# kobigurk/phase2-bn254

Measured on AMD Instinct MI355X. Metric: BN254 G1 MSM throughput (Mscalar-mul/s) at 2^26 points, higher is better.
Workload: dtype u32x8 (256-bit Montgomery limbs)

## Files before the change

phase2-bn254_amd/csrc/msm_common.hpp:

```cpp
#pragma once
#include <stdint.h>

namespace zk {

constexpr uint32_t SIGN_BIT = 0x80000000u;

struct MsmGeom {
  uint32_t c;
  uint32_t W;
  uint32_t nb;
  uint8_t width[64];
  uint8_t shift[64];
  uint32_t rmul;
  uint32_t rshift;
};

constexpr uint32_t MSM_SIZE_BINS = 4096;
constexpr uint32_t PART_THREADS = 1024;
constexpr uint32_t PART_MAX_ST = 16384;
constexpr uint32_t PART_MAX_EB = PART_MAX_ST / PART_THREADS;
constexpr uint32_t PART_LO_MAX = 12;
constexpr uint32_t PART_EC = 32;
constexpr uint32_t PART_LDS_A = 76 * 1024;
constexpr uint32_t PART_LDS_MAX = 160 * 1024 - 512;
constexpr uint32_t KEY_NONE_MASK = 0x00ffffffu;

struct PartGeom {
  uint32_t lo_bits;
  uint32_t nbin;
  uint32_t st;
  uint32_t n_st;
  uint32_t n_chunk;
  uint32_t rows_per_chunk;
};

constexpr uint32_t BIG_SEG = PART_EC * PART_THREADS;

struct BigPlan {
  uint32_t n_big;
  uint32_t total_seg;
};

constexpr uint32_t MSM_HEAVY_BLOCKS = 65536;
constexpr uint32_t MSM_HEAVY_SEG = 4096;
constexpr uint32_t MSM_HEAVY_LANES = 64;
constexpr uint32_t MSM_PAIR_MAX_BUCKETS = 3u << 17;

constexpr uint32_t MSM_FINAL_MAX = 1024;
constexpr uint32_t MSM_TREE_SLICE = 512;
constexpr uint32_t MSM_MAX_LEVELS = 8;
constexpr uint32_t MSM_MAX_JOBS = MSM_MAX_LEVELS + 24;

}
```

phase2-bn254_amd/csrc/msm_host.hpp:

```cpp
#pragma once
#include <atomic>
#include <chrono>
#include <cstring>
#include <map>
#include <mutex>
#include <type_traits>
#include <vector>

#include "msm_impl.hpp"
#include "msm_join.hpp"
#include "msm_partition.hpp"
#include "msm_plan.hpp"
#include "msm_pools.hpp"

namespace zk {

namespace {

std::mutex g_part_cfg_mu;
std::map<int, int> g_part_cfg;
template <class F>
int part_configure(int dev) {
  std::lock_guard<std::mutex> lk(g_part_cfg_mu);
  auto it = g_part_cfg.find(dev);
  if (it != g_part_cfg.end()) return it->second;
  int rc = zk::part_configure(dev);
  hipError_t e = hipFuncSetAttribute(reinterpret_cast<const void*>(msm_tree_kernel<F>), hipFuncAttributeMaxDynamicSharedMemorySize, 160 * 1024);
  if (e != hipSuccess) {
    std::fprintf(stderr, "[mi355zk] hipFuncSetAttribute(partition kernel, 160 KiB LDS) failed: %s\n", hipGetErrorString(e));
    rc = ZK_ERR_DEVICE;
  }
  g_part_cfg[dev] = rc;
  return rc;
}

template <class F>
struct MsmWs : MsmPartWs {
  XYZZ<F>*seg_sums, *buckets, *partA, *partS, *rc, *wsums, *sumtmp;
  static_assert(sizeof(XYZZ<F>) == (sizeof(F) == sizeof(Fq) ? 128 : 256), "msm_plan.hpp sizes the record regions by these");
  MsmWs(char* ws, const MsmLayout& L) : MsmPartWs(ws, L) {
    at(ws, seg_sums, L.seg_sums), at(ws, buckets, L.buckets), at(ws, partA, L.partA), at(ws, partS, L.partS), at(ws, rc, L.rc), at(ws, wsums, L.wsums);
    at(ws, sumtmp, L.sumtmp);
  }
};

template <class F>
struct MsmCall : MsmPartCall {
  MsmWs<F> ws;
  bool dense;
};

template <class Fn>
void with_a4_carry(bool a4, bool carry, Fn&& fn) {
  auto with_carry = [&](auto A4) { if (carry) fn(A4, std::true_type{}); else fn(A4, std::false_type{}); };
  if (a4) with_carry(std::true_type{}); else with_carry(std::false_type{});
}

struct HeavyParams {
  uint32_t hb, heavy, seg, grid;
  int dense, carry;
};
template <class F>
int launch_heavy(hipStream_t st, const Affine<F>* bases, const uint32_t* vals, const uint32_t* first, const uint32_t* last, const uint32_t* order,
                 const uint32_t* sizes_b, uint32_t* item_off, XYZZ<F>* seg_sums, XYZZ<F>* buckets, unsigned long long* d_err, const HeavyParams& H) {
  launch_heavy_plan(st, sizes_b, H.hb, H.heavy, H.seg, item_off);
  ZK_HIP(hipGetLastError());
  hipLaunchKernelGGL(msm_accumulate_heavy_kernel<F>, dim3(H.grid), dim3(MSM_HEAVY_LANES), MSM_HEAVY_LANES * sizeof(typename BucketAcc<F>::type), st, bases, vals,
                     first, last, order, item_off, H.hb, H.seg, seg_sums, H.dense, d_err);
  ZK_HIP(hipGetLastError());
  hipLaunchKernelGGL(msm_heavy_combine_kernel<F>, dim3(H.hb < 2048 ? H.hb : 2048), dim3(64), 64 * sizeof(typename BucketAcc<F>::type), st, seg_sums, order, item_off,
                     H.hb, buckets, H.carry);
  ZK_HIP(hipGetLastError());
  return ZK_OK;
}

template <class F>
int launch_accumulate(const MsmCall<F>& A, const ChunkPlan& C, const Affine<F>* bases_set, bool carry) {
  constexpr bool g2 = std::is_same<F, Fq2>::value;
  const MsmWs<F>& W = A.ws;
  const MsmKnobs& K = A.knobs;
  const hipStream_t st = A.st;
  const uint32_t n_buckets = A.plan.n_buckets;
// ... 18 lines not shown
  const bool pair = pair_mode < 0 ? n_buckets <= MSM_PAIR_MAX_BUCKETS : pair_mode != 0;
  const bool w2 = g2 && !pair && (K.g2_waves == 0 ? g_msm_inflight[A.dev & 15].load(std::memory_order_relaxed) <= 1 : K.g2_waves == 2);
  with_a4_carry(K.acc_a4, carry, [&](auto A4, auto CARRY) {
    constexpr bool a4 = decltype(A4)::value, cy = decltype(CARRY)::value;
    auto go = [&](auto kern, dim3 g) {
      hipLaunchKernelGGL(kern, g, block, 0, st, bases_set, W.vals_b, W.first, W.last, W.order, skip_len, skip_hb, n_buckets, W.buckets, dense, W.d_err);
    };
    if constexpr (g2) {
      if (pair) go(msm_accumulate_pair_kernel<a4, cy>, pgrid);
      else if (w2) go(msm_accumulate_g2w2_kernel<a4, cy>, grid);
      else go(msm_accumulate_kernel<F, a4, cy>, grid);
    } else {
      if (pair) go(msm_accumulate_pair_g1_kernel<a4, cy>, pgrid);
      else go(msm_accumulate_kernel<F, a4, cy>, grid);
    }
  });
  ZK_HIP(hipGetLastError());
  prof_end(msm_slots().acc, st);
  if (msm_checkpoint(A, "accumulate", C)) return (int)ZK_ERR_DEVICE;
  return ZK_OK;
}

template <class F>
int launch_reduce(const MsmCall<F>& A) {
  const MsmPlan& P = A.plan;
  const MsmWs<F>& W = A.ws;
  const hipStream_t st = A.st;
  const uint32_t WL = P.WL, n_levels = P.n_levels, n_out = P.n_out, t_rows = P.t_rows, t_cols = P.t_cols;
  TreeJobs<F> J{};
  J.quad = A.knobs.quad_tail ? 1u : 0u;
  const XYZZ<F>* in = W.buckets;
  uint64_t o = 0;
  for (uint32_t lv = 0; lv < n_levels; ++lv) {
    uint32_t threads = P.lvl_chunks[lv] * WL;
    XYZZ<F>* LA = W.partA + o * WL;
    XYZZ<F>* LS = W.partS + o * WL;
    if (A.knobs.quad_tail && threads <= A.knobs.quad_max_chunks)
      hipLaunchKernelGGL(msm_reduce_level_quad_kernel<F>, dim3((4 * threads + 255) / 256), dim3(256), 0, st, in, P.lvl_cnt[lv], 1u << P.lvl_logl[lv],
                         lv == 0 ? 1u : 0u, WL, LA, LS);
    else
      hipLaunchKernelGGL(msm_reduce_level_kernel<F>, dim3((threads + 255) / 256), dim3(256), 0, st, in, P.lvl_cnt[lv], 1u << P.lvl_logl[lv],
                         lv == 0 ? 1u : 0u, WL, LA, LS);
    ZK_HIP(hipGetLastError());
    J.in[lv] = LA;
    J.cnt[lv] = J.stride[lv] = P.lvl_chunks[lv];
    J.bit[lv] = -1;
    in = LS;
    o += P.lvl_chunks[lv];
  }
  auto plain = [&J](uint32_t j) { J.reps[j] = 1; J.rep_stride[j] = 0; J.elem_stride[j] = 1; J.limit[j] = 0xffffffffu; J.off[j] = 0; };
  for (uint32_t lv = 0; lv < n_levels; ++lv) plain(lv);
  uint32_t n_jobs = n_levels;
  if (!P.tail2d) {
    for (uint32_t j = 0; j < P.final_bits; ++j, ++n_jobs) {
      plain(n_jobs);
      J.in[n_jobs] = in;
      J.cnt[n_jobs] = J.stride[n_jobs] = P.final_cnt;
      J.bit[n_jobs] = (int32_t)j;
      J.off[n_jobs] = P.final_off;
    }
  } else {
    J.in[n_jobs] = in; J.cnt[n_jobs] = t_cols; J.stride[n_jobs] = P.final_cnt; J.bit[n_jobs] = -1; J.off[n_jobs] = 0;
    J.reps[n_jobs] = t_rows; J.rep_stride[n_jobs] = t_cols; J.elem_stride[n_jobs] = 1; J.limit[n_jobs] = P.final_cnt;
    ++n_jobs;
    J.in[n_jobs] = in; J.cnt[n_jobs] = t_rows; J.stride[n_jobs] = P.final_cnt; J.bit[n_jobs] = -1; J.off[n_jobs] = 0;
    J.reps[n_jobs] = t_cols; J.rep_stride[n_jobs] = 1; J.elem_stride[n_jobs] = t_cols; J.limit[n_jobs] = P.final_cnt;
    ++n_jobs;
  }
  const size_t lds = 256 * sizeof(typename BucketAcc<F>::type);
  XYZZ<F>* dst = W.sumtmp;
  for (uint32_t launch = 0;; ++launch) {
    const bool families = P.tail2d && launch == 0;
    uint32_t left = 1;
    uint64_t o_dst = 0;
    for (uint32_t j = 0; j < n_jobs; ++j) {
      const uint32_t sl = (J.cnt[j] + MSM_TREE_SLICE - 1) / MSM_TREE_SLICE;
      J.first_block[j + 1] = J.first_block[j] + J.reps[j] * sl;
      if (sl > left) left = sl;
    }
    const bool last = left == 1 && !families;
    for (uint32_t j = 0; j < n_jobs; ++j) {
      const uint32_t sl = (J.cnt[j] + MSM_TREE_SLICE - 1) / MSM_TREE_SLICE;
      if (families && j >= n_levels) {
        J.out[j] = W.rc + (j == n_levels ? 0 : t_rows);
        J.out_w[j] = t_rows + t_cols;
      } else if (last) {
        J.out[j] = W.wsums + j;
        J.out_w[j] = n_out;
      } else {
        J.out[j] = dst + o_dst;
        J.out_w[j] = 1;
        o_dst += (uint64_t)WL * sl;
      }
    }
    J.n_jobs = n_jobs;
    hipLaunchKernelGGL(msm_tree_kernel<F>, dim3(J.first_block[n_jobs] * WL), dim3(256), lds, st, J);
    ZK_HIP(hipGetLastError());
    if (last) break;
    for (uint32_t j = 0; j < (families ? n_levels : n_jobs); ++j) {
      const uint32_t sl = (J.cnt[j] + MSM_TREE_SLICE - 1) / MSM_TREE_SLICE;
      J.in[j] = J.out[j];
      J.cnt[j] = J.stride[j] = sl;
      J.bit[j] = -1;
      plain(j);
    }
    if (families) {
      n_jobs = n_levels;
      for (uint32_t j = 0; j < P.final_bits; ++j, ++n_jobs) {
        plain(n_jobs);
        J.in[n_jobs] = W.rc + t_rows;
        J.cnt[n_jobs] = t_cols;
        J.stride[n_jobs] = t_rows + t_cols;
        J.bit[n_jobs] = (int32_t)j;
        J.off[n_jobs] = P.final_off;
      }
      for (uint32_t j = 0; j < P.row_bits; ++j, ++n_jobs) {
        plain(n_jobs);
        J.in[n_jobs] = W.rc;
        J.cnt[n_jobs] = t_rows;
        J.stride[n_jobs] = t_rows + t_cols;
        J.bit[n_jobs] = (int32_t)j;
      }
    }
    dst = dst == W.sumtmp ? W.sumtmp + (uint64_t)WL * P.tree_tmp : W.sumtmp;
  }
  return ZK_OK;
}

template <class F>
int msm_finish_set(const MsmCall<F>& A, SmallWsLease& lease, std::unique_lock<std::mutex>& lk, const Affine<F>* d_bases, const uint32_t* d_sc_first,
                   Jacobian<F>* result, bool last_set, long long* err_index_out) {
  const MsmPlan& P = A.plan;
  const hipStream_t st = A.st;
// ... 62 lines not shown
  if (top) ZK_HIP(hipMemcpyAsync(T.vals.data(), A.ws.vals_b, (size_t)top * 4, hipMemcpyDeviceToHost, A.st));
  ZK_HIP(hipStreamSynchronize(A.st));
  return ZK_OK;
}

template <class F>
int msm_device(const Affine<F>* d_bases, uint64_t n_bases, uint64_t base_offset, const uint32_t* d_scalars, uint64_t n,
               const uint32_t* d_density, const uint32_t* d_dprefix, hipStream_t st, Jacobian<F>* out, long long* err_index_out,
               bool dense = false, const Affine<F>* d_bases2 = nullptr, Jacobian<F>* out2 = nullptr, uint32_t wgroups = 1,
               uint32_t wgroup = 0, bool scalars_mont = false, MsmChunks* chunks = nullptr, uint64_t table_stride = 0, uint32_t table_c = 0) {
  *out = Jacobian<F>::zero();
  if (out2) *out2 = Jacobian<F>::zero();
  *err_index_out = -1;
  if (n == 0) return ZK_OK;
  if (n_bases > 0x7fffffffull || n > 0x7fffffffull) return ZK_ERR_BAD_ARGS;
  int dev = 0;
  ZK_HIP(hipGetDevice(&dev));
  struct Inflight {
    std::atomic<int>& c;
    explicit Inflight(std::atomic<int>& x) : c(x) { c.fetch_add(1, std::memory_order_relaxed); }
    ~Inflight() { c.fetch_sub(1, std::memory_order_relaxed); }
  } inflight(g_msm_inflight[dev & 15]);
  const MsmKnobs K = msm_knobs();
  MsmRequest R;
  R.group = (int)(sizeof(F) / sizeof(Fq));
  R.n = n;
  R.base_offset = base_offset;
  R.wgroups = wgroups;
  R.wgroup = wgroup;
  if (chunks) R.n_chunks = chunks->n_chunks, R.cuts = chunks->cuts;
  R.two_sets = d_bases2 != nullptr;
  R.table_stride = table_stride;
  R.table_c = table_c;
  const MsmPlan P = msm_plan(R, K);
  if (P.rc) return P.rc;

  int rc = part_configure<F>(dev);
  if (rc) return rc;
  Workspace& dev_ws = ws_of(dev);
  std::unique_lock<std::mutex> lk(dev_ws.mu, std::defer_lock);
  void* base = nullptr;
  SmallWsLease lease;
  if (P.L.total_bytes <= WS_SMALL) {
    rc = tws_acquire(dev, P.L.total_bytes, st, &lease, &base);
  } else {
    lk.lock();
    rc = ws_reserve(dev_ws, P.L.total_bytes, &base);
  }
  if (rc) return rc;
  const MsmCall<F> A{{P, K, R.group, dev, st, n, base_offset, table_stride, d_density, d_dprefix, scalars_mont}, MsmWs<F>((char*)base, P.L), dense};
  ZK_HIP(hipMemsetAsync(A.ws.d_err, 0xff, 16, st));
  lease.idle = false;

  const uint32_t* d_sc_first = d_scalars;
  for (uint32_t c = 0; c < (uint32_t)P.chunks.size(); ++c) {
    const ChunkPlan& C = P.chunks[c];
    const uint32_t* d_sc = d_scalars;
    if (chunks) {
      const void* p = nullptr;
      rc = chunks->acquire(c, st, &p);
      if (rc) return rc;
      d_sc = (const uint32_t*)p;
    }
    d_sc_first = d_sc;
    rc = launch_digits(A, A.ws, C, d_sc);
    if (rc == ZK_OK && chunks) rc = chunks->digits_enqueued(c, st);
    if (rc == ZK_OK) rc = launch_partition(A, A.ws, C);
    if (rc == ZK_OK) rc = launch_accumulate(A, C, d_bases, c > 0);
    if (rc) return rc;
  }
  if (g_msm_bucket_tap) {
    if (P.chunks.size() != 1) return ZK_ERR_BAD_ARGS;
    if (int trc = msm_tap_buckets(A, *g_msm_bucket_tap)) return trc;
  }
  const bool two_sets = d_bases2 != nullptr && out2 != nullptr;
  rc = msm_finish_set(A, lease, lk, d_bases, d_sc_first, out, !two_sets, err_index_out);
  if (rc != ZK_OK || !two_sets) return rc;
  lease.idle = false;
  rc = launch_accumulate(A, P.chunks[0], d_bases2, false);
  if (rc) return rc;
  return msm_finish_set(A, lease, lk, d_bases, d_sc_first, out2, true, err_index_out);
}

// ... 52 lines not shown
```

phase2-bn254_amd/csrc/msm_impl.hpp:

```cpp
#pragma once
#include <hip/hip_runtime.h>

#include <type_traits>

#include "curveu.hpp"
#include "device_util.hpp"
#include "msm_common.hpp"

namespace zk {

namespace {

template <class F>
__device__ __forceinline__ Affine<F> load_affine(const Affine<F>* p) {
  Affine<F> r;
  const uint4* q = reinterpret_cast<const uint4*>(p);
  uint4* d = reinterpret_cast<uint4*>(&r);
#pragma unroll
  for (int i = 0; i < (int)(sizeof(Affine<F>) / 16); ++i) d[i] = q[i];
  return r;
}

template <class T>
__device__ __forceinline__ void store_vec(T* p, const T& v) {
// ... 287 lines not shown
    const Affine<Fq2>* __restrict__ bases, const uint32_t* __restrict__ vals, const uint32_t* __restrict__ first, const uint32_t* __restrict__ last,
    const uint32_t* __restrict__ order, uint32_t heavy, uint32_t hb, uint32_t n_buckets, XYZZ<Fq2>* __restrict__ buckets, int skip_zero,
    unsigned long long* __restrict__ err_base) {
  accumulate_pair_body<Fq2, A4, CARRY>(bases, vals, first, last, order, heavy, hb, n_buckets, buckets, skip_zero, err_base);
}
template <bool A4, bool CARRY>
__global__ void __launch_bounds__(256) msm_accumulate_pair_g1_kernel(
    const Affine<Fq>* __restrict__ bases, const uint32_t* __restrict__ vals, const uint32_t* __restrict__ first, const uint32_t* __restrict__ last,
    const uint32_t* __restrict__ order, uint32_t heavy, uint32_t hb, uint32_t n_buckets, XYZZ<Fq>* __restrict__ buckets, int skip_zero,
    unsigned long long* __restrict__ err_base) {
  accumulate_pair_body<Fq, A4, CARRY>(bases, vals, first, last, order, heavy, hb, n_buckets, buckets, skip_zero, err_base);
}

template <class F>
__global__ void __launch_bounds__(256) __attribute__((amdgpu_waves_per_eu(1, 2))) msm_accumulate_split_kernel(
    const Affine<F>* __restrict__ bases, const uint32_t* __restrict__ vals, const uint32_t* __restrict__ first, const uint32_t* __restrict__ last,
    const uint32_t* __restrict__ order, uint32_t split_t, uint32_t heavy, uint32_t heavy_hb, uint32_t hb, XYZZ<F>* __restrict__ buckets,
    int skip_zero, unsigned long long* __restrict__ err_base) {
  using U = typename BucketAcc<F>::type;
  const uint32_t gt = blockIdx.x * blockDim.x + threadIdx.x, i = gt >> 2, role = gt & 3u;
  if (i >= hb) return;
  const uint32_t b = order[i];
  const uint32_t j = first[b], e = last[b];
  if (e - j <= split_t || (e - j > heavy && i < heavy_hb)) return;
  U part = xyzzr_load(XYZZ<F>::zero());
  if (j + role < e) part = xyzzr_load(xyzzu_to_r(accumulate_run<F, false>(U::zero(), bases, vals, j + role, e, 4, skip_zero != 0, err_base)));
  const U p0 = quad_fetch<0>(part), p1 = quad_fetch<1>(part), p2 = quad_fetch<2>(part), p3 = quad_fetch<3>(part);
  const U sum = xyzzr_add_quad(xyzzr_add_quad(p0, p1, role), xyzzr_add_quad(p2, p3, role), role);
  if (role == 0) store_vec(buckets + b, xyzzr_store(sum));
}

template <class F>
__global__ void __launch_bounds__(256) msm_reduce_level_kernel(const XYZZ<F>* __restrict__ in, uint32_t count, uint32_t L, uint32_t off,
                                                              uint32_t W, XYZZ<F>* __restrict__ outA, XYZZ<F>* __restrict__ outS) {
  uint32_t chunks = (count + L - 1) / L;
  uint32_t t = blockIdx.x * blockDim.x + threadIdx.x;
  if (t >= chunks * W) return;
  uint32_t w = t / chunks, ch = t % chunks;
  uint32_t lo = ch * L, hi = lo + L < count ? lo + L : count;
  const XYZZ<F>* B = in + (uint64_t)w * count;
  uint32_t steps = 2 * (hi - lo);
  auto run = xyzzr_load(XYZZ<F>::zero()), acc = run;
  for (uint32_t it = 0; it < steps; ++it) {
    uint32_t x = hi - 1 - (it >> 1);
    bool do_acc = ((it & 1) != 0) == (off != 0);
    auto a = do_acc ? acc : run;
    auto b = do_acc ? run : xyzzr_load(load_vec(B + x));
    xyzzr_add(a, b);
    if (do_acc) acc = a;
    else run = a;
  }
  store_vec(outA + t, xyzzr_store(acc));
  store_vec(outS + t, xyzzr_store(run));
}

template <class F>
__global__ void __launch_bounds__(256) __attribute__((amdgpu_waves_per_eu(1, 2))) msm_reduce_level_quad_kernel(const XYZZ<F>* __restrict__ in, uint32_t count, uint32_t L, uint32_t off,
                                                                   uint32_t W, XYZZ<F>* __restrict__ outA, XYZZ<F>* __restrict__ outS) {
  const uint32_t chunks = (count + L - 1) / L;
  const uint32_t gt = blockIdx.x * blockDim.x + threadIdx.x, t = gt >> 2, role = gt & 3u;
  if (t >= chunks * W) return;
  const uint32_t w = t / chunks, ch = t % chunks;
  const uint32_t lo = ch * L, hi = lo + L < count ? lo + L : count;
  const XYZZ<F>* B = in + (uint64_t)w * count;
  auto run = xyzzr_load(XYZZ<F>::zero()), acc = run;
  for (uint32_t x = hi; x-- > lo;) {
    run = xyzzr_add_quad(run, xyzzr_load(load_vec(B + x)), role);
    if (off != 0 || x > lo) acc = xyzzr_add_quad(acc, run, role);
  }
  if (role == 0) store_vec(outA + t, xyzzr_store(acc));
  if (role == 1) store_vec(outS + t, xyzzr_store(run));
}

template <class F>
struct TreeJobs {
  const XYZZ<F>* in[MSM_MAX_JOBS];
  XYZZ<F>* out[MSM_MAX_JOBS];
  uint32_t cnt[MSM_MAX_JOBS];
  uint32_t stride[MSM_MAX_JOBS];
  uint32_t reps[MSM_MAX_JOBS], rep_stride[MSM_MAX_JOBS], elem_stride[MSM_MAX_JOBS], limit[MSM_MAX_JOBS];
  uint32_t out_w[MSM_MAX_JOBS];
  uint32_t off[MSM_MAX_JOBS];
  int32_t bit[MSM_MAX_JOBS];
  uint32_t first_block[MSM_MAX_JOBS + 1];
  uint32_t n_jobs;
  uint32_t quad;
};
template <class F>
__global__ void __launch_bounds__(256) __attribute__((amdgpu_waves_per_eu(1, 2))) msm_tree_kernel(const TreeJobs<F> J) {
  extern __shared__ __attribute__((aligned(16))) unsigned char smem[];
  using U = typename BucketAcc<F>::type;
  U* sh = reinterpret_cast<U*>(smem);
  const uint32_t per_w = J.first_block[J.n_jobs];
  const uint32_t w = blockIdx.x / per_w, r = blockIdx.x % per_w;
  uint32_t job = 0;
  while (job + 1 < J.n_jobs && J.first_block[job + 1] <= r) ++job;
  const uint32_t count = J.cnt[job];
  const uint32_t slices = (count + MSM_TREE_SLICE - 1) / MSM_TREE_SLICE;
  const uint32_t idx = r - J.first_block[job];
  const uint32_t rp = idx / slices, slice = idx % slices;
  const int32_t bit = J.bit[job];
  const uint32_t off = J.off[job], es = J.elem_stride[job];
  const uint32_t rbase = rp * J.rep_stride[job], limit = J.limit[job];
  const XYZZ<F>* P = J.in[job] + (uint64_t)w * J.stride[job] + rbase;
  const uint32_t x0 = slice * MSM_TREE_SLICE + threadIdx.x, x1 = x0 + 256;
  XYZZ<F> r0 = XYZZ<F>::zero(), r1 = XYZZ<F>::zero();
  if (x0 < count && (uint64_t)rbase + (uint64_t)x0 * es < limit && (bit < 0 || (((x0 + off) >> bit) & 1))) r0 = load_vec(P + (uint64_t)x0 * es);
  if (x1 < count && (uint64_t)rbase + (uint64_t)x1 * es < limit && (bit < 0 || (((x1 + off) >> bit) & 1))) r1 = load_vec(P + (uint64_t)x1 * es);
  U acc = xyzzr_load(r0), other = xyzzr_load(r1);
  const uint32_t quad_from = J.quad ? 128u : 0u;
  for (uint32_t s = 256;;) {
    xyzzr_add(acc, other);
    s >>= 1;
    if (s == 0 || s < quad_from) break;
    if (threadIdx.x >= s && threadIdx.x < 2 * s) sh[threadIdx.x] = acc;
    __syncthreads();
    other = threadIdx.x < s ? sh[threadIdx.x + s] : U::zero();
  }
  {
    if (quad_from) {
      if (threadIdx.x < 128) sh[threadIdx.x] = acc;
      __syncthreads();
      const uint32_t q = threadIdx.x >> 2, role = threadIdx.x & 3u;
      acc = sh[q];
      for (uint32_t s = 64; s > 0; s >>= 1) {
        if (q < s) {
          acc = xyzzr_add_quad(acc, sh[q + s], role);
          if (role == 0) sh[q] = acc;
        }
        __syncthreads();
      }
    }
  }
  if (threadIdx.x == 0) store_vec(J.out[job] + ((uint64_t)w * J.out_w[job] + rp) * slices + slice, xyzzr_store(acc));
}

template <class F>
__global__ void __launch_bounds__(256) msm_identity_scan_kernel(const Affine<F>* __restrict__ bases, const uint32_t* __restrict__ scalars, uint64_t n,
                                                               uint64_t base_offset, const uint32_t* __restrict__ density,
                                                               const uint32_t* __restrict__ dprefix, unsigned long long* __restrict__ err_base) {
  const uint64_t i = (uint64_t)blockIdx.x * blockDim.x + threadIdx.x;
  if (i >= n) return;
  uint64_t bi = base_offset + i;
  if (density != nullptr) {
    const uint32_t wd = density[i >> 5];
// ... 19 lines not shown
```

phase2-bn254_amd/csrc/msm_plan.hpp:

```cpp
#pragma once
#include <algorithm>
#include <cmath>
#include <cstdio>
#include <cstdlib>
#include <vector>

#include "host_util.hpp"
#include "msm_common.hpp"

namespace zk {

struct MsmKnobs {
  int msm_c = 0;
  uint32_t radix_m = 0, radix_s = 0;
  bool radix_off = false;
  int table_c = 0;
  int part_lo = -1, part_st = 0;
  bool no_tail2d = false;
  bool no_small_scan = false;
  bool debug = false;
  bool fused_a = false;
  uint32_t part_xcds = 8;
  bool acc_a4 = true;
  int g1_pair = -1, g2_pair = -1;
  int g2_waves = 0;
  bool quad_tail = true;
  uint32_t quad_max_chunks = 65536;
  bool trace_join = false;
  bool join_serial = false;
  uint32_t final_max = MSM_FINAL_MAX;
  uint8_t logl[MSM_MAX_LEVELS] = {};
  bool split_off = false;
  uint32_t split_t = 0;
};

inline MsmKnobs msm_knobs() {
  static const MsmKnobs process = [] {
    MsmKnobs K;
    auto num = [](const char* name, int unset) { const char* s = std::getenv(name); return s ? std::atoi(s) : unset; };
    auto set = [](const char* name) { return std::getenv(name) != nullptr; };
    K.msm_c = num("MI355ZK_MSM_C", 0);
    if (const char* s = std::getenv("MI355ZK_MSM_RADIX")) {
      int rm = 0, rs = 0;
      if (std::sscanf(s, "%d,%d", &rm, &rs) == 2 && rm >= 3 && rm <= 15 && (rm & 1) && rs >= 2 && rs <= 22) K.radix_m = (uint32_t)rm, K.radix_s = (uint32_t)rs;
      K.radix_off = s[0] == '0';
    }
    K.table_c = num("MI355ZK_MSM_TABLE_C", 0);
    K.part_lo = num("MI355ZK_PART_LO", -1);
    K.part_st = num("MI355ZK_PART_ST", 0);
    K.no_tail2d = set("MI355ZK_MSM_NO_TAIL2D");
    K.no_small_scan = set("MI355ZK_MSM_NO_SMALL_SCAN");
    K.debug = set("MI355ZK_DEBUG");
    K.fused_a = set("MI355ZK_PART_FUSED_A");
    K.part_xcds = num("MI355ZK_PART_XCDS", 0) >= 1 ? (uint32_t)num("MI355ZK_PART_XCDS", 0) : 8u;
    K.acc_a4 = !set("MI355ZK_ACC_NARROW");
    auto tri = [](const char* name) { const char* s = std::getenv(name); return !s ? -1 : s[0] == '0' ? 0 : 1; };
    K.g1_pair = tri("MI355ZK_G1_PAIR");
    K.g2_pair = tri("MI355ZK_G2_PAIR");
    if (const char* s = std::getenv("MI355ZK_G2_WAVES")) K.g2_waves = s[0] == '1' ? 1 : 2;
    if (const char* s = std::getenv("MI355ZK_MSM_QUAD")) K.quad_tail = s[0] != '0';
    if (const char* s = std::getenv("MI355ZK_MSM_QUAD_MAX")) K.quad_max_chunks = (uint32_t)std::atoi(s);
    K.trace_join = set("MI355ZK_TRACE_MSM");
    K.join_serial = set("MI355ZK_MSM_JOIN_SERIAL");
    return K;
  }();
  MsmKnobs K = process;
  if (const char* s = std::getenv("MI355ZK_MSM_FINAL_MAX"))
    if (std::atoi(s) >= 64) K.final_max = (uint32_t)std::atoi(s);
  if (const char* s = std::getenv("MI355ZK_MSM_LOGL")) {
    for (uint32_t lv = 0; lv < MSM_MAX_LEVELS; ++lv) {
      uint32_t k = 0;
      const char* q = s;
      while (k < lv && *q) { if (*q == ',') ++k; ++q; }
      if (k == lv && *q >= '1' && *q <= '5') K.logl[lv] = (uint8_t)(*q - '0');
    }
  }
  if (const char* s = std::getenv("MI355ZK_MSM_SPLIT")) {
    K.split_off = s[0] == '0' && s[1] == 0;
    if (std::atoi(s) > 0) K.split_t = (uint32_t)std::atoi(s);
  }
  return K;
}

inline size_t align_up(size_t x, size_t a = 256) { return (x + a - 1) / a * a; }

inline MsmGeom make_geom(uint32_t c) {
  MsmGeom G{};
  G.rmul = 1;
  G.c = c;
  uint32_t W = 1;
  while ((W - 1) * c + (c - 1) < 254) ++W;
  G.W = W;
  G.nb = 1u << (c - 1);
  uint32_t top = c - 1;
  if (W == 1) top = 254 < top ? 254 : top;
  uint32_t rest = 254 > top ? 254 - top : 0;
  uint32_t base = W > 1 ? rest / (W - 1) : 0, rem = W > 1 ? rest % (W - 1) : 0;
  uint32_t bit = 0;
  for (uint32_t w = 0; w + 1 < W; ++w) {
    G.width[w] = (uint8_t)(base + (w < rem ? 1 : 0));
    G.shift[w] = (uint8_t)bit;
    bit += G.width[w];
  }
  G.width[W - 1] = (uint8_t)(254 - bit);
  G.shift[W - 1] = (uint8_t)bit;
  return G;
}

inline MsmGeom make_geom_radix(uint32_t rmul, uint32_t rshift) {
// ... 73 lines not shown
  auto pop = [&](uint32_t lo) { return (uint64_t)n * (1ull << lo) / nb; };
  uint32_t lo = lo_cap;
  const uint64_t pop_target = 12288;
  const uint64_t pop_cap = (uint64_t)PART_EC * PART_THREADS * 85 / 100;
  while (lo > 0 && pop(lo) > pop_target && fits_lds(lo - 1, PART_LDS_A)) --lo;
  while (lo > 0 && pop(lo) > pop_cap && fits(lo - 1)) --lo;
  while (!fits(lo) && lo < PART_LO_MAX) ++lo;
  if (K.part_lo >= 0 && K.part_lo <= (int)lo_cap && fits((uint32_t)K.part_lo)) lo = (uint32_t)K.part_lo;
  P.lo_bits = lo;
  P.nbin = nbin_of(lo);
  uint32_t st = PART_MAX_ST;
  while (st > PART_THREADS && (n / st) * WL < 256) st >>= 1;
  if (K.part_st >= (int)PART_THREADS && K.part_st <= (int)PART_MAX_ST && K.part_st % (int)PART_THREADS == 0) st = (uint32_t)K.part_st;
  while (st > PART_THREADS && (uint64_t)st * 8 + (uint64_t)P.nbin * 8 + 256 > PART_LDS_MAX) st -= PART_THREADS;
  if ((uint64_t)st * 8 + (uint64_t)P.nbin * 8 + 256 > PART_LDS_MAX) st = 0;
  P.st = st;
  P.n_st = (uint32_t)((n + st - 1) / st);
  P.rows_per_chunk = P.n_st > 64 ? (P.n_st + 63) / 64 : 1;
  P.n_chunk = (P.n_st + P.rows_per_chunk - 1) / P.rows_per_chunk;
  return P;
}


struct MsmRequest {
  int group = 1;
  uint64_t n = 0;
  uint64_t base_offset = 0;
  uint32_t wgroups = 1, wgroup = 0;
  uint32_t n_chunks = 1;
  const uint64_t* cuts = nullptr;
  bool two_sets = false;
  uint64_t table_stride = 0;
  uint32_t table_c = 0;
};

struct ChunkPlan {
  uint64_t lo, n, m, np;
  PartGeom P;
  uint32_t ncell, heavy, heavy_seg, hb, max_items;
  bool small_scan;
  uint32_t split_t, split_hb;
};

struct MsmLayout {
  size_t keys, pairs, tile_hist, tile_off, csum, total, bin_start, out_start;
  size_t gcnt, gcur, big_col, big_seg, big_plan;
  size_t first, last, hist, sizes_b, ids_b, item_off, seg_sums, buckets, partA, partS;
  size_t rc;
  size_t wsums;
  size_t err;
  size_t sumtmp;
  size_t total_bytes;
  size_t back_bytes() const { return (err - wsums) + 16; }
};

struct MsmPlan {
  int rc = ZK_OK;
  int group = 1;
  bool tmode = false;
  MsmGeom G{};
  uint32_t WD = 0, w_lo = 0, w_hi = 0;
  uint32_t WL = 0;
  uint32_t n_buckets = 0;
  uint64_t m_max = 0;
  uint32_t n_levels = 0, lvl_cnt[MSM_MAX_LEVELS + 1] = {}, lvl_chunks[MSM_MAX_LEVELS + 1] = {}, lvl_logl[MSM_MAX_LEVELS + 1] = {};
  uint64_t total_chunks = 1;
  uint32_t final_cnt = 0;
  uint32_t final_off = 0;
  bool tail2d = false;
  uint32_t cols_log = 0, t_cols = 0, t_rows = 0;
  uint32_t final_bits = 1;
  uint32_t row_bits = 0;
  uint32_t n_out = 0, e_k[MSM_MAX_JOBS] = {}, e_max = 0;
  uint32_t tree_cnt = 0;
  uint64_t tree_tmp = 0;
  std::vector<ChunkPlan> chunks;
  MsmLayout L{};
};

inline int msm_plan_fill(const MsmRequest& R, const MsmKnobs& K, MsmPlan& P) {
  const uint64_t n = R.n;
  const bool g1 = R.group == 1;
  const size_t rec_bytes = g1 ? 128 : 256;
  P.group = R.group;
  if (R.wgroups == 0 || R.wgroup >= R.wgroups) return ZK_ERR_BAD_ARGS;
  const bool tmode = P.tmode = R.table_stride != 0;
  if (tmode && (R.wgroups != 1 || R.n_chunks != 1 || R.two_sets || R.table_c < 4 || R.table_c > 24 || R.base_offset > R.table_stride)) return ZK_ERR_BAD_ARGS;
  const uint64_t whole[2] = {0, n};
  const uint32_t n_chunks = R.n_chunks;
  const uint64_t* cuts = R.cuts ? R.cuts : whole;
  if (n_chunks == 0 || (R.cuts == nullptr && n_chunks != 1) || cuts[0] != 0 || cuts[n_chunks] != n) return ZK_ERR_BAD_ARGS;
  if (n_chunks > 1 && R.two_sets) return ZK_ERR_BAD_ARGS;
  uint64_t n_max = 0;
  for (uint32_t c = 0; c < n_chunks; ++c) {
    if (cuts[c + 1] <= cuts[c] || (c > 0 && (cuts[c] & 31))) return ZK_ERR_BAD_ARGS;
    if (cuts[c + 1] - cuts[c] > n_max) n_max = cuts[c + 1] - cuts[c];
  }
  const MsmGeom G = P.G = tmode ? make_geom(R.table_c) : choose_geom(n, R.group, R.wgroups, K);
  if (G.W == 0 || G.W % R.wgroups) return ZK_ERR_BAD_ARGS;
  const uint32_t WD = P.WD = G.W / R.wgroups;
  P.w_lo = R.wgroup * WD;
  P.w_hi = P.w_lo + WD;
  const uint32_t WL = P.WL = tmode ? 1u : WD;
  if (tmode && (uint64_t)G.W * R.table_stride > 0x7fffffffull) return ZK_ERR_BAD_ARGS;
  const uint64_t m_max = P.m_max = tmode ? ((n_max + 3) & ~3ull) * WD : n_max * WL;
  if (m_max > 0xfffffff0ull) return ZK_ERR_BAD_ARGS;
  const uint32_t n_buckets = P.n_buckets = WL * G.nb;
  uint32_t final_cnt = G.nb, n_levels = 0;
  auto tail_fits = [&](uint32_t cnt) { return !K.no_tail2d && g1 && (uint64_t)cnt * WL <= (1ull << 17) && cnt >= (1u << 15) && cnt <= (1u << 18); };
  while (final_cnt > K.final_max && n_levels < MSM_MAX_LEVELS) {
    if (tail_fits(final_cnt)) break;
    uint32_t logl = (uint64_t)final_cnt * WL >= (1ull << 20) ? 3 : 2;
    if (K.logl[n_levels]) logl = K.logl[n_levels];
    P.lvl_cnt[n_levels] = final_cnt;
    P.lvl_logl[n_levels] = logl;
    P.lvl_chunks[n_levels] = (final_cnt + (1u << logl) - 1) >> logl;
    P.total_chunks += P.lvl_chunks[n_levels];
    final_cnt = P.lvl_chunks[n_levels];
    ++n_levels;
  }
  P.n_levels = n_levels;
  P.final_cnt = final_cnt;
  const uint32_t final_off = P.final_off = n_levels == 0 ? 1u : 0u;
  const bool tail2d = P.tail2d = tail_fits(final_cnt);
  if (tail2d) {
    uint32_t lg = 0;
    while ((1u << lg) < final_cnt) ++lg;
    P.cols_log = (lg + 1) / 2;
  }
  const uint32_t t_cols = P.t_cols = tail2d ? 1u << P.cols_log : final_cnt, t_rows = P.t_rows = tail2d ? (final_cnt + t_cols - 1) / t_cols : 0;
  while ((1u << P.final_bits) <= t_cols - 1 + final_off) ++P.final_bits;
  while (t_rows > 1 && (1u << P.row_bits) <= t_rows - 1) ++P.row_bits;

  P.chunks.resize(n_chunks);
  uint64_t keys_cap = 0, tile_hist_b = 0, tile_off_b = 0, csum_b = 0;
  uint32_t ncell_max = 0, hb_max = 0, items_max = 0;
  for (uint32_t c = 0; c < n_chunks; ++c) {
    ChunkPlan& C = P.chunks[c];
    C.lo = cuts[c];
    C.n = cuts[c + 1] - cuts[c];
    C.np = tmode ? ((C.n + 3) & ~3ull) * WD : C.n;
    C.m = C.np * WL;
    C.P = choose_part(C.np, WL, G.nb, K);
    if (C.P.st == 0) return ZK_ERR_BAD_ARGS;
    C.ncell = WL * C.P.nbin;
    C.small_scan = !K.no_small_scan && (uint64_t)C.P.n_st * C.ncell <= (1u << 16);
    const uint64_t vals_cap = C.m + 3ull * n_buckets + 4ull * C.ncell + 4;
    if (vals_cap > 0xfffffff0ull) return ZK_ERR_BAD_ARGS;
    keys_cap = std::max(keys_cap, vals_cap);
    tile_hist_b = std::max<uint64_t>(tile_hist_b, (uint64_t)C.P.n_st * ((C.ncell + 1) & ~1u) * 2);
// ... 75 lines not shown
```

Before: 1015.

## Size reduce-level spans and tree elements-per-lane to device residency

At configure time the code queries the CU count and the occupancy of the reduce-level and tree kernels. It uses the resulting residency to let each tree-kernel lane fold more than two elements, doubling elements-per-lane on the largest job until the total workgroup count fits in one resident wave. Optionally, enabled only through an environment variable, each reduce-level lane walks several adjacent chunks serially and carries the weighted accumulator across them, so fewer lanes write partial sums. The aim is to cut tail-wave waste and the number of partial records the later tree passes must merge. The cost is longer serial add chains per lane and less parallelism when the grid was not oversubscribed.

```diff
diff --git a/phase2-bn254_amd/csrc/msm_common.hpp b/phase2-bn254_amd/csrc/msm_common.hpp
--- a/phase2-bn254_amd/csrc/msm_common.hpp
+++ b/phase2-bn254_amd/csrc/msm_common.hpp
@@ -48,6 +48,9 @@
 
 constexpr uint32_t MSM_FINAL_MAX = 1024;
 constexpr uint32_t MSM_TREE_SLICE = 512;
+constexpr uint32_t MSM_TREE_LANES = 256;
+constexpr uint32_t MSM_TREE_MAX_EPL = 8;
+constexpr uint32_t MSM_MAX_SPAN = 8;
 constexpr uint32_t MSM_MAX_LEVELS = 8;
 constexpr uint32_t MSM_MAX_JOBS = MSM_MAX_LEVELS + 24;
 
diff --git a/phase2-bn254_amd/csrc/msm_host.hpp b/phase2-bn254_amd/csrc/msm_host.hpp
--- a/phase2-bn254_amd/csrc/msm_host.hpp
+++ b/phase2-bn254_amd/csrc/msm_host.hpp
@@ -17,21 +17,41 @@
 
 namespace {
 
+struct MsmDeviceCfg {
+  int rc = ZK_OK;
+  uint32_t level_lanes = 0;
+  uint32_t level_quads = 0;
+  uint32_t tree_slots = 0;
+};
 std::mutex g_part_cfg_mu;
-std::map<int, int> g_part_cfg;
-template <class F>
-int part_configure(int dev) {
+std::map<int, MsmDeviceCfg> g_part_cfg;
+template <class F>
+MsmDeviceCfg part_configure(int dev) {
   std::lock_guard<std::mutex> lk(g_part_cfg_mu);
   auto it = g_part_cfg.find(dev);
   if (it != g_part_cfg.end()) return it->second;
-  int rc = zk::part_configure(dev);
+  MsmDeviceCfg C;
+  C.rc = zk::part_configure(dev);
   hipError_t e = hipFuncSetAttribute(reinterpret_cast<const void*>(msm_tree_kernel<F>), hipFuncAttributeMaxDynamicSharedMemorySize, 160 * 1024);
   if (e != hipSuccess) {
     std::fprintf(stderr, "[mi355zk] hipFuncSetAttribute(partition kernel, 160 KiB LDS) failed: %s\n", hipGetErrorString(e));
-    rc = ZK_ERR_DEVICE;
-  }
-  g_part_cfg[dev] = rc;
-  return rc;
+    C.rc = ZK_ERR_DEVICE;
+  }
+  int cus = 0;
+  if (hipDeviceGetAttribute(&cus, hipDeviceAttributeMultiprocessorCount, dev) != hipSuccess || cus < 0) cus = 0;
+  auto resident = [&](const void* kern, size_t lds) {
+    int blocks = 0;
+    if (hipOccupancyMaxActiveBlocksPerMultiprocessor(&blocks, kern, 256, lds) != hipSuccess || blocks < 0) blocks = 0, (void)hipGetLastError();
+    return (uint32_t)blocks * (uint32_t)cus;
+  };
+  C.level_lanes = resident(reinterpret_cast<const void*>(msm_reduce_level_kernel<F>), 0) * 256;
+  C.level_quads = resident(reinterpret_cast<const void*>(msm_reduce_level_quad_kernel<F>), 0) * 64;
+  C.tree_slots = resident(reinterpret_cast<const void*>(msm_tree_kernel<F>), MSM_TREE_LANES * sizeof(typename BucketAcc<F>::type));
+  if (msm_knobs().trace_join)
+    std::fprintf(stderr, "[mi355zk] reduce residency (group %d, device %d, %d CUs): %u level lanes, %u level quads, %u tree workgroups\n",
+                 (int)(sizeof(F) / sizeof(Fq)), dev, cus, C.level_lanes, C.level_quads, C.tree_slots);
+  g_part_cfg[dev] = C;
+  return C;
 }
 
 template <class F>
@@ -48,6 +68,7 @@
 struct MsmCall : MsmPartCall {
   MsmWs<F> ws;
   bool dense;
+  uint32_t tree_slots;
 };
 
 template <class Fn>
@@ -132,18 +153,18 @@
   const XYZZ<F>* in = W.buckets;
   uint64_t o = 0;
   for (uint32_t lv = 0; lv < n_levels; ++lv) {
-    uint32_t threads = P.lvl_chunks[lv] * WL;
+    uint32_t threads = P.lvl_alanes[lv] * WL;
     XYZZ<F>* LA = W.partA + o * WL;
     XYZZ<F>* LS = W.partS + o * WL;
-    if (A.knobs.quad_tail && threads <= A.knobs.quad_max_chunks)
+    if (P.lvl_quad[lv])
       hipLaunchKernelGGL(msm_reduce_level_quad_kernel<F>, dim3((4 * threads + 255) / 256), dim3(256), 0, st, in, P.lvl_cnt[lv], 1u << P.lvl_logl[lv],
-                         lv == 0 ? 1u : 0u, WL, LA, LS);
+                         lv == 0 ? 1u : 0u, WL, P.lvl_span[lv], LA, LS);
     else
       hipLaunchKernelGGL(msm_reduce_level_kernel<F>, dim3((threads + 255) / 256), dim3(256), 0, st, in, P.lvl_cnt[lv], 1u << P.lvl_logl[lv],
-                         lv == 0 ? 1u : 0u, WL, LA, LS);
+                         lv == 0 ? 1u : 0u, WL, P.lvl_span[lv], LA, LS);
     ZK_HIP(hipGetLastError());
     J.in[lv] = LA;
-    J.cnt[lv] = J.stride[lv] = P.lvl_chunks[lv];
+    J.cnt[lv] = J.stride[lv] = P.lvl_alanes[lv];
     J.bit[lv] = -1;
     in = LS;
     o += P.lvl_chunks[lv];
@@ -173,14 +194,18 @@
     const bool families = P.tail2d && launch == 0;
     uint32_t left = 1;
     uint64_t o_dst = 0;
+    bool plain_sum[MSM_MAX_JOBS];
+    for (uint32_t j = 0; j < n_jobs; ++j) plain_sum[j] = J.bit[j] < 0;
+    msm_tree_epl_fill(n_jobs, J.cnt, J.reps, plain_sum, WL, A.tree_slots, A.knobs.tree_epl, J.epl);
+    auto slices_of = [&J](uint32_t j) { return (J.cnt[j] + MSM_TREE_LANES * J.epl[j] - 1) / (MSM_TREE_LANES * J.epl[j]); };
     for (uint32_t j = 0; j < n_jobs; ++j) {
-      const uint32_t sl = (J.cnt[j] + MSM_TREE_SLICE - 1) / MSM_TREE_SLICE;
+      const uint32_t sl = slices_of(j);
       J.first_block[j + 1] = J.first_block[j] + J.reps[j] * sl;
       if (sl > left) left = sl;
     }
     const bool last = left == 1 && !families;
     for (uint32_t j = 0; j < n_jobs; ++j) {
-      const uint32_t sl = (J.cnt[j] + MSM_TREE_SLICE - 1) / MSM_TREE_SLICE;
+      const uint32_t sl = slices_of(j);
       if (families && j >= n_levels) {
         J.out[j] = W.rc + (j == n_levels ? 0 : t_rows);
         J.out_w[j] = t_rows + t_cols;
@@ -198,7 +223,7 @@
     ZK_HIP(hipGetLastError());
     if (last) break;
     for (uint32_t j = 0; j < (families ? n_levels : n_jobs); ++j) {
-      const uint32_t sl = (J.cnt[j] + MSM_TREE_SLICE - 1) / MSM_TREE_SLICE;
+      const uint32_t sl = slices_of(j);
       J.in[j] = J.out[j];
       J.cnt[j] = J.stride[j] = sl;
       J.bit[j] = -1;
@@ -327,11 +352,13 @@
   R.two_sets = d_bases2 != nullptr;
   R.table_stride = table_stride;
   R.table_c = table_c;
+  const MsmDeviceCfg cfg = part_configure<F>(dev);
+  if (cfg.rc) return cfg.rc;
+  if (K.span_rule) R.reduce_cap = cfg.level_lanes, R.reduce_cap_quads = cfg.level_quads;
   const MsmPlan P = msm_plan(R, K);
   if (P.rc) return P.rc;
 
-  int rc = part_configure<F>(dev);
-  if (rc) return rc;
+  int rc = ZK_OK;
   Workspace& dev_ws = ws_of(dev);
   std::unique_lock<std::mutex> lk(dev_ws.mu, std::defer_lock);
   void* base = nullptr;
@@ -343,7 +370,7 @@
     rc = ws_reserve(dev_ws, P.L.total_bytes, &base);
   }
   if (rc) return rc;
-  const MsmCall<F> A{{P, K, R.group, dev, st, n, base_offset, table_stride, d_density, d_dprefix, scalars_mont}, MsmWs<F>((char*)base, P.L), dense};
+  const MsmCall<F> A{{P, K, R.group, dev, st, n, base_offset, table_stride, d_density, d_dprefix, scalars_mont}, MsmWs<F>((char*)base, P.L), dense, cfg.tree_slots};
   ZK_HIP(hipMemsetAsync(A.ws.d_err, 0xff, 16, st));
   lease.idle = false;
 
diff --git a/phase2-bn254_amd/csrc/msm_impl.hpp b/phase2-bn254_amd/csrc/msm_impl.hpp
--- a/phase2-bn254_amd/csrc/msm_impl.hpp
+++ b/phase2-bn254_amd/csrc/msm_impl.hpp
@@ -343,44 +343,54 @@
 
 template <class F>
 __global__ void __launch_bounds__(256) msm_reduce_level_kernel(const XYZZ<F>* __restrict__ in, uint32_t count, uint32_t L, uint32_t off,
-                                                              uint32_t W, XYZZ<F>* __restrict__ outA, XYZZ<F>* __restrict__ outS) {
-  uint32_t chunks = (count + L - 1) / L;
-  uint32_t t = blockIdx.x * blockDim.x + threadIdx.x;
-  if (t >= chunks * W) return;
-  uint32_t w = t / chunks, ch = t % chunks;
-  uint32_t lo = ch * L, hi = lo + L < count ? lo + L : count;
+                                                              uint32_t W, uint32_t span, XYZZ<F>* __restrict__ outA, XYZZ<F>* __restrict__ outS) {
+  const uint32_t chunks = (count + L - 1) / L, alanes = (chunks + span - 1) / span;
+  const uint32_t t = blockIdx.x * blockDim.x + threadIdx.x;
+  if (t >= alanes * W) return;
+  const uint32_t w = t / alanes, a_idx = t % alanes;
+  const uint32_t ch_lo = a_idx * span, ch_hi = ch_lo + span < chunks ? ch_lo + span : chunks;
   const XYZZ<F>* B = in + (uint64_t)w * count;
-  uint32_t steps = 2 * (hi - lo);
-  auto run = xyzzr_load(XYZZ<F>::zero()), acc = run;
-  for (uint32_t it = 0; it < steps; ++it) {
-    uint32_t x = hi - 1 - (it >> 1);
-    bool do_acc = ((it & 1) != 0) == (off != 0);
-    auto a = do_acc ? acc : run;
-    auto b = do_acc ? run : xyzzr_load(load_vec(B + x));
-    xyzzr_add(a, b);
-    if (do_acc) acc = a;
-    else run = a;
+  XYZZ<F>* S = outS + (uint64_t)w * chunks;
+  auto acc = xyzzr_load(XYZZ<F>::zero());
+  for (uint32_t ch = ch_hi; ch-- > ch_lo;) {
+    const uint32_t lo = ch * L, hi = lo + L < count ? lo + L : count;
+    const uint32_t steps = 2 * (hi - lo);
+    auto run = xyzzr_load(XYZZ<F>::zero());
+    for (uint32_t it = 0; it < steps; ++it) {
+      uint32_t x = hi - 1 - (it >> 1);
+      bool do_acc = ((it & 1) != 0) == (off != 0);
+      auto a = do_acc ? acc : run;
+      auto b = do_acc ? run : xyzzr_load(load_vec(B + x));
+      xyzzr_add(a, b);
+      if (do_acc) acc = a;
+      else run = a;
+    }
+    store_vec(S + ch, xyzzr_store(run));
   }
   store_vec(outA + t, xyzzr_store(acc));
-  store_vec(outS + t, xyzzr_store(run));
 }
 
 template <class F>
 __global__ void __launch_bounds__(256) __attribute__((amdgpu_waves_per_eu(1, 2))) msm_reduce_level_quad_kernel(const XYZZ<F>* __restrict__ in, uint32_t count, uint32_t L, uint32_t off,
-                                                                   uint32_t W, XYZZ<F>* __restrict__ outA, XYZZ<F>* __restrict__ outS) {
-  const uint32_t chunks = (count + L - 1) / L;
+                                                                   uint32_t W, uint32_t span, XYZZ<F>* __restrict__ outA, XYZZ<F>* __restrict__ outS) {
+  const uint32_t chunks = (count + L - 1) / L, alanes = (chunks + span - 1) / span;
   const uint32_t gt = blockIdx.x * blockDim.x + threadIdx.x, t = gt >> 2, role = gt & 3u;
-  if (t >= chunks * W) return;
-  const uint32_t w = t / chunks, ch = t % chunks;
-  const uint32_t lo = ch * L, hi = lo + L < count ? lo + L : count;
+  if (t >= alanes * W) return;
+  const uint32_t w = t / alanes, a_idx = t % alanes;
+  const uint32_t ch_lo = a_idx * span, ch_hi = ch_lo + span < chunks ? ch_lo + span : chunks;
   const XYZZ<F>* B = in + (uint64_t)w * count;
-  auto run = xyzzr_load(XYZZ<F>::zero()), acc = run;
-  for (uint32_t x = hi; x-- > lo;) {
-    run = xyzzr_add_quad(run, xyzzr_load(load_vec(B + x)), role);
-    if (off != 0 || x > lo) acc = xyzzr_add_quad(acc, run, role);
+  XYZZ<F>* S = outS + (uint64_t)w * chunks;
+  auto acc = xyzzr_load(XYZZ<F>::zero());
+  for (uint32_t ch = ch_hi; ch-- > ch_lo;) {
+    const uint32_t lo = ch * L, hi = lo + L < count ? lo + L : count;
+    auto run = xyzzr_load(XYZZ<F>::zero());
+    for (uint32_t x = hi; x-- > lo;) {
+      run = xyzzr_add_quad(run, xyzzr_load(load_vec(B + x)), role);
+      if (off != 0 || x > lo) acc = xyzzr_add_quad(acc, run, role);
+    }
+    if (role == 1) store_vec(S + ch, xyzzr_store(run));
   }
   if (role == 0) store_vec(outA + t, xyzzr_store(acc));
-  if (role == 1) store_vec(outS + t, xyzzr_store(run));
 }
 
 template <class F>
@@ -396,7 +406,9 @@
   uint32_t first_block[MSM_MAX_JOBS + 1];
   uint32_t n_jobs;
   uint32_t quad;
+  uint8_t epl[MSM_MAX_JOBS];
 };
+static_assert(sizeof(TreeJobs<Fq>) <= 4096 && sizeof(TreeJobs<Fq2>) <= 4096, "TreeJobs travels as a kernel argument");
 template <class F>
 __global__ void __launch_bounds__(256) __attribute__((amdgpu_waves_per_eu(1, 2))) msm_tree_kernel(const TreeJobs<F> J) {
   extern __shared__ __attribute__((aligned(16))) unsigned char smem[];
@@ -407,21 +419,30 @@
   uint32_t job = 0;
   while (job + 1 < J.n_jobs && J.first_block[job + 1] <= r) ++job;
   const uint32_t count = J.cnt[job];
-  const uint32_t slices = (count + MSM_TREE_SLICE - 1) / MSM_TREE_SLICE;
+  const uint32_t epl = J.epl[job], slice_len = MSM_TREE_LANES * epl;
+  const uint32_t slices = (count + slice_len - 1) / slice_len;
   const uint32_t idx = r - J.first_block[job];
   const uint32_t rp = idx / slices, slice = idx % slices;
   const int32_t bit = J.bit[job];
   const uint32_t off = J.off[job], es = J.elem_stride[job];
   const uint32_t rbase = rp * J.rep_stride[job], limit = J.limit[job];
   const XYZZ<F>* P = J.in[job] + (uint64_t)w * J.stride[job] + rbase;
-  const uint32_t x0 = slice * MSM_TREE_SLICE + threadIdx.x, x1 = x0 + 256;
-  XYZZ<F> r0 = XYZZ<F>::zero(), r1 = XYZZ<F>::zero();
-  if (x0 < count && (uint64_t)rbase + (uint64_t)x0 * es < limit && (bit < 0 || (((x0 + off) >> bit) & 1))) r0 = load_vec(P + (uint64_t)x0 * es);
-  if (x1 < count && (uint64_t)rbase + (uint64_t)x1 * es < limit && (bit < 0 || (((x1 + off) >> bit) & 1))) r1 = load_vec(P + (uint64_t)x1 * es);
-  U acc = xyzzr_load(r0), other = xyzzr_load(r1);
+  const uint32_t x0 = slice * slice_len + threadIdx.x;
+  auto fetch = [&](uint32_t k) {
+    const uint32_t x = x0 + MSM_TREE_LANES * k;
+    XYZZ<F> rec = XYZZ<F>::zero();
+    if (x < count && (uint64_t)rbase + (uint64_t)x * es < limit && (bit < 0 || (((x + off) >> bit) & 1))) rec = load_vec(P + (uint64_t)x * es);
+    return xyzzr_load(rec);
+  };
+  U acc = fetch(0), other = fetch(1);
   const uint32_t quad_from = J.quad ? 128u : 0u;
+  uint32_t k = 2;
   for (uint32_t s = 256;;) {
     xyzzr_add(acc, other);
+    if (k < epl) {
+      other = fetch(k++);
+      continue;
+    }
     s >>= 1;
     if (s == 0 || s < quad_from) break;
     if (threadIdx.x >= s && threadIdx.x < 2 * s) sh[threadIdx.x] = acc;
diff --git a/phase2-bn254_amd/csrc/msm_plan.hpp b/phase2-bn254_amd/csrc/msm_plan.hpp
--- a/phase2-bn254_amd/csrc/msm_plan.hpp
+++ b/phase2-bn254_amd/csrc/msm_plan.hpp
@@ -32,6 +32,9 @@
   uint8_t logl[MSM_MAX_LEVELS] = {};
   bool split_off = false;
   uint32_t split_t = 0;
+  uint8_t span[MSM_MAX_LEVELS] = {};
+  bool span_rule = false;
+  uint32_t tree_epl = 0;
 };
 
 inline MsmKnobs msm_knobs() {
@@ -75,6 +78,20 @@
       if (k == lv && *q >= '1' && *q <= '5') K.logl[lv] = (uint8_t)(*q - '0');
     }
   }
+  if (const char* s = std::getenv("MI355ZK_MSM_SPAN")) {
+    const char* q = s;
+    K.span_rule = s[0] == 'a';
+    for (uint32_t lv = 0; lv < MSM_MAX_LEVELS && *q; ++lv) {
+      const int v = std::atoi(q);
+      if (v >= 1) K.span[lv] = (uint8_t)(v > (int)MSM_MAX_SPAN ? (int)MSM_MAX_SPAN : v);
+      while (*q && *q != ',') ++q;
+      if (*q == ',') ++q;
+    }
+  }
+  if (const char* s = std::getenv("MI355ZK_MSM_TREE_EPL")) {
+    const int v = std::atoi(s);
+    if (v == 2 || v == 4 || v == 8) K.tree_epl = (uint32_t)v;
+  }
   if (const char* s = std::getenv("MI355ZK_MSM_SPLIT")) {
     K.split_off = s[0] == '0' && s[1] == 0;
     if (std::atoi(s) > 0) K.split_t = (uint32_t)std::atoi(s);
@@ -214,6 +231,7 @@
   bool two_sets = false;
   uint64_t table_stride = 0;
   uint32_t table_c = 0;
+  uint32_t reduce_cap = 0, reduce_cap_quads = 0;
 };
 
 struct ChunkPlan {
@@ -246,6 +264,8 @@
   uint32_t n_buckets = 0;
   uint64_t m_max = 0;
   uint32_t n_levels = 0, lvl_cnt[MSM_MAX_LEVELS + 1] = {}, lvl_chunks[MSM_MAX_LEVELS + 1] = {}, lvl_logl[MSM_MAX_LEVELS + 1] = {};
+  uint32_t lvl_span[MSM_MAX_LEVELS + 1] = {}, lvl_alanes[MSM_MAX_LEVELS + 1] = {};
+  bool lvl_quad[MSM_MAX_LEVELS + 1] = {};
   uint64_t total_chunks = 1;
   uint32_t final_cnt = 0;
   uint32_t final_off = 0;
@@ -259,6 +279,33 @@
   std::vector<ChunkPlan> chunks;
   MsmLayout L{};
 };
+
+inline uint32_t msm_span_for(uint32_t WL, uint32_t chunks, uint32_t cap) {
+  if (cap == 0) return 1;
+  auto gens = [&](uint32_t lanes_per_w) { return ((uint64_t)WL * lanes_per_w + cap - 1) / cap; };
+  const uint64_t now = gens(chunks);
+  for (uint32_t g = MSM_MAX_SPAN; g > 1; --g)
+    if (gens((chunks + g - 1) / g) * g <= now) return g;
+  return 1;
+}
+
+inline void msm_tree_epl_fill(uint32_t n_jobs, const uint32_t* cnt, const uint32_t* reps, const bool* plain, uint32_t WL, uint32_t slots, uint32_t forced,
+                              uint8_t* epl) {
+  auto slices = [&](uint32_t j) { return (cnt[j] + MSM_TREE_LANES * epl[j] - 1) / (MSM_TREE_LANES * epl[j]); };
+  auto wgs = [&](uint32_t j) { return (uint64_t)reps[j] * slices(j); };
+  for (uint32_t j = 0; j < n_jobs; ++j) epl[j] = (uint8_t)(plain[j] && forced ? forced : 2u);
+  if (forced || slots == 0) return;
+  for (;;) {
+    uint64_t total = 0;
+    uint32_t best = n_jobs;
+    for (uint32_t j = 0; j < n_jobs; ++j) {
+      total += wgs(j) * WL;
+      if (plain[j] && epl[j] < MSM_TREE_MAX_EPL && slices(j) > 1 && (best == n_jobs || wgs(j) > wgs(best))) best = j;
+    }
+    if (total <= slots || best == n_jobs) return;
+    epl[best] = (uint8_t)(epl[best] * 2);
+  }
+}
 
 inline int msm_plan_fill(const MsmRequest& R, const MsmKnobs& K, MsmPlan& P) {
   const uint64_t n = R.n;
@@ -298,6 +345,13 @@
     P.lvl_logl[n_levels] = logl;
     P.lvl_chunks[n_levels] = (final_cnt + (1u << logl) - 1) >> logl;
     P.total_chunks += P.lvl_chunks[n_levels];
+    const uint32_t chunks = P.lvl_chunks[n_levels];
+    const bool quad = P.lvl_quad[n_levels] = K.quad_tail && (uint64_t)chunks * WL <= K.quad_max_chunks;
+    uint32_t span = msm_span_for(WL, chunks, quad ? (R.reduce_cap_quads ? R.reduce_cap_quads : R.reduce_cap / 4) : R.reduce_cap);
+    if (K.span[n_levels]) span = K.span[n_levels] > MSM_MAX_SPAN ? MSM_MAX_SPAN : K.span[n_levels];
+    if (span > chunks) span = chunks;
+    P.lvl_span[n_levels] = span;
+    P.lvl_alanes[n_levels] = (chunks + span - 1) / span;
     final_cnt = P.lvl_chunks[n_levels];
     ++n_levels;
   }
```

Measured after the change: 1017 (median of 6 runs). About the same (+0.3%).
